# yusong-yan/MultiRaft

Hardware: AMD Instinct MI355X
Metric: quorum commit decisions/sec @64k groups×5 peers; % HBM roofline (higher is better)
Workload: dtype int32

## Files before the change

multiraft_amd/csrc/mraft_abi_msg.hip:

```cpp
#include <vector>

#include "mraft_engine.h"

using namespace mraft::host;

extern "C" {

int mraft_gather_append_args(mraft_engine *h, const int32_t *slots, const int32_t *peers,
                             int64_t n, mraft_ae_args *out_args, int32_t *item_err, int32_t where) {
  TRY(enter(h));
  if (n < 0 || (n > 0 && (!slots || !peers || !out_args || !item_err)))
    return fail(MRAFT_E_INVAL, "null argument");
  if (n == 0) return MRAFT_OK;
  Stage sg(h, where);
  const int32_t *s = sg.in(slots, n), *p = sg.in(peers, n);
  mraft_ae_args *o = sg.out(out_args, n);
  int32_t *e = sg.out(item_err, n);
  TRY(sg.status());
  mraft::launch_gather_args(dev_of(h), s, p, n, o, e, h->stream);
  return sg.finish();
}

int mraft_handle_append_entries(mraft_engine *h, const mraft_ae_args *args, int64_t n,
                                const int32_t *entry_terms, int64_t n_entry_terms,
                                mraft_ae_reply *replies, int32_t *item_err, int32_t where) {
  return mraft_handle_append_entries_ex(h, args, n, entry_terms, n_entry_terms, replies, nullptr, item_err, where);
}

int mraft_handle_append_entries_ex(mraft_engine *h, const mraft_ae_args *args, int64_t n,
                                   const int32_t *entry_terms, int64_t n_entry_terms,
                                   mraft_ae_reply *replies, mraft_ae_result *results, int32_t *item_err,
                                   int32_t where) {
  TRY(enter(h));
  if (n < 0 || (n > 0 && (!args || !replies || !item_err)))
    return fail(MRAFT_E_INVAL, "null argument");
  if (n > INT32_MAX) return fail(MRAFT_E_INVAL, "n = %lld items exceeds 2^31 - 1", (long long)n);
  if (entry_terms && n_entry_terms < 0) return fail(MRAFT_E_INVAL, "n_entry_terms < 0");
  if (n == 0) return MRAFT_OK;
  TRY(ensure_claim(h));
  Stage sg(h, where);
  const mraft_ae_args *a = sg.in(args, n);
  const int32_t *en = sg.in(entry_terms, entry_terms ? n_entry_terms : 0);
  mraft_ae_reply *r = sg.out(replies, n);
  mraft_ae_result *rs = sg.out(results, n);
  int32_t *e = sg.out(item_err, n);
  TRY(sg.status());
  if (en) {
    claim(h, a, n, nullptr, e);
    mraft::launch_handle_ae_host(dev_of(h), a, n, en, n_entry_terms, r, e, rs, h->stream);
    return sg.finish();
  }
  if (!h->ae_total) TRY(alloc_async(h, &h->ae_total, mraft::kAeTotalWords, "AppendEntries counters", true));
  const size_t nn = (size_t)n;
  mraft::HsArgs ka{};
  ka.s = dev_of(h); ka.args = a; ka.n = n; ka.rep = r; ka.err = e; ka.res = rs;
  ka.total = h->ae_total; ka.claim = h->claim; ka.srcmark = h->srcmark; ka.epoch = h->epoch;
  uint8_t *sethd;
  TRY(scratch(h, kScrAeSoff, nn, &ka.soff));
  TRY(scratch(h, kScrAeSetHead, nn, &sethd));
  ka.sethd = sethd;
  TRY(scratch(h, kScrAeDefer, nn * mraft::kAeStripes, &ka.defer));
  const long long last_nd = hint(h, kHintDeferred);
  const long long gmin = h->defer_grid_min;
  const int grid = (int)(last_nd < gmin ? gmin : last_nd > kDeferGridMax ? kDeferGridMax : last_nd);
  ka.nslot = (int)std::min<int64_t>(grid, std::max<int64_t>(1, kCycSlotWords / h->L));
  void *order;
  TRY(scratch_bytes(h, kScrAeOrder, mraft::ae_order_carve(ka, nullptr), &order));
  mraft::ae_order_carve(ka, order);
  TRY(scratch_zeroed(h, kScrAeKin, nn, &ka.kin));
  ka.hint = h->dhint_dev;
  if (h->stage_auto) {
    const long long need = hint(h, kHintStageNeed);
    if (need > h->stage_cap)
      h->stage_cap = std::min<int64_t>((int64_t)INT32_MAX, (need + need / 4 + kStageStep - 1) / kStageStep * kStageStep);
  }
  if (h->stage_cap > 0 && scratch(h, kScrAeStage, (size_t)h->stage_cap, &ka.stage) != MRAFT_OK) {
    ka.stage = nullptr;
    h->stage_auto = false;
  }
  ka.stage_cap = ka.stage ? h->stage_cap : 0;
  const int ni = h->P - 1 < 1 ? 1 : h->P - 1 > 7 ? 7 : h->P - 1;
  const int64_t n_log = gp_of(h) * h->L;
  mraft::launch_claim_ae(a, n, n_log, h->L, gp_of(h), ni, h->claim, h->srcmark, h->epoch, e, sethd, h->ae_total,
                         h->stream);
  mraft::launch_handle_ae_ref(ka, ni, grid, h->stream);
  return sg.finish();
}

int mraft_set_stage_capacity(mraft_engine *h, int64_t words) {
  TRY(enter(h));
  if (words == MRAFT_STAGE_AUTO) {
    h->stage_auto = true;
    return MRAFT_OK;
  }
  if (words < 0 || words > INT32_MAX) return fail(MRAFT_E_INVAL, "stage capacity %lld out of [0, 2^31)", (long long)words);
  h->stage_cap = words;
  h->stage_auto = false;
  return MRAFT_OK;
}

int64_t mraft_get_stage_capacity(const mraft_engine *h) { return h ? h->stage_cap : -1; }

int mraft_process_append_replies(mraft_engine *h, const mraft_ae_result *items, int64_t n,
                                 const int64_t *seg_begin, int64_t n_seg, int32_t *out_flags,
                                 int32_t *item_err, int32_t where) {
  return fold_replies(h, items, n, seg_begin, n_seg, out_flags, item_err, where, [=](const FoldBufs<mraft_ae_result> &b) -> int {
    void *sc;
    TRY(scratch_bytes(h, kScrFoldScan, mraft::fold_scan_bytes(n, b.ns), &sc));
    mraft::launch_fold(dev_of(h), b.it, n, b.sb, b.ns, gp_of(h), h->claim, h->epoch, b.se, b.fl, b.e, sc, h->stream);
    return MRAFT_OK;
  });
}

int mraft_start(mraft_engine *h, const int32_t *slots, const int32_t *counts, int64_t n,
                int32_t *out_index, int32_t *out_term, int32_t *out_is_leader, int32_t *item_err,
                int32_t where) {
  TRY(enter(h));
  if (n < 0 || (n > 0 && (!slots || !out_index || !out_term || !out_is_leader || !item_err)))
    return fail(MRAFT_E_INVAL, "null argument");
  if (n == 0) return MRAFT_OK;
  TRY(ensure_claim(h));
  Stage sg(h, where);
  const int32_t *s = sg.in(slots, n), *c = sg.in(counts, n);
  int32_t *oi = sg.out(out_index, n), *ot = sg.out(out_term, n), *ol = sg.out(out_is_leader, n);
  int32_t *e = sg.out(item_err, n);
  TRY(sg.status());
  mraft::launch_start(dev_of(h), s, c, n, oi, ot, ol, e, h->claim, h->epoch, h->stream);
  return sg.finish();
}

int mraft_collect_apply(mraft_engine *h, int32_t *out_from, int32_t *out_to, int32_t *out_snap_index,
                        int32_t *out_snap_term, int32_t where) {
  TRY(enter(h));
  if (!out_from || !out_to) return fail(MRAFT_E_INVAL, "null argument");
  if (!out_snap_index != !out_snap_term) return fail(MRAFT_E_INVAL, "snapshot outputs: both or neither");
  Stage sg(h, where);
  const size_t gp = (size_t)gp_of(h);
  int32_t *f = sg.out(out_from, gp), *t = sg.out(out_to, gp);
  int32_t *si = sg.out(out_snap_index, gp), *st = sg.out(out_snap_term, gp);
  TRY(sg.status());
  mraft::launch_collect_apply(dev_of(h), f, t, si, st, h->stream);
  return sg.finish();
}

int mraft_collect_apply_compact(mraft_engine *h, int32_t *out_slots, int32_t *out_snap_index,
                                int32_t *out_snap_term, int32_t *out_from, int32_t *out_to, int64_t cap,
                                int64_t *out_n, int32_t where) {
  TRY(enter(h));
  if (cap < 0 || !out_n || (cap > 0 && (!out_slots || !out_from || !out_to)) ||
      (!out_snap_index) != (!out_snap_term))
    return fail(MRAFT_E_INVAL, "null argument");
  Stage sg(h, where);
  int32_t *sl = sg.out(out_slots, cap), *si = sg.out(out_snap_index, cap), *stm = sg.out(out_snap_term, cap);
  int32_t *f = sg.out(out_from, cap), *t = sg.out(out_to, cap), *bc;
  int64_t *total = sg.out(out_n, 1);
  TRY(sg.status());
  TRY(scratch(h, kScrApplyBlocks, (size_t)((gp_of(h) + 255) / 256), &bc));
  mraft::launch_collect_apply_compact(dev_of(h), bc, cap, sl, si, stm, f, t, total, h->stream);
  return sg.finish();
}

int mraft_snapshot(mraft_engine *h, const int32_t *slots, const int32_t *index, int64_t n,
                   int32_t *item_err, int32_t where) {
  TRY(enter(h));
  if (n < 0 || (n > 0 && (!slots || !index || !item_err))) return fail(MRAFT_E_INVAL, "null argument");
  if (n == 0) return MRAFT_OK;
  TRY(ensure_claim(h));
  Stage sg(h, where);
  const int32_t *s = sg.in(slots, n), *x = sg.in(index, n);
  int32_t *e = sg.out(item_err, n);
  TRY(sg.status());
  claim(h, s, n, nullptr, e);
  mraft::launch_snapshot(dev_of(h), s, x, n, e, h->stream);
  return sg.finish();
}

int mraft_gather_install_snapshot_args(mraft_engine *h, const int32_t *slots, const int32_t *peers,
                                       int64_t n, mraft_is_args *out_args, int32_t *item_err,
// ... 184 lines not shown
```

multiraft_amd/csrc/mraft_engine.h:

```cpp
#pragma once
#include <hip/hip_runtime.h>

#include <cstddef>
#include <cstdint>

#include "../../include/mraft.h"
#include "mraft_device.h"
#include "mraft_internal.h"

constexpr int kMaxShards = 8;
constexpr int64_t kDefaultStageWords = (int64_t)1 << 22;
#ifndef MRAFT_DEFER_GRID_MIN
#define MRAFT_DEFER_GRID_MIN 512
#endif
constexpr int kDeferGridMin = MRAFT_DEFER_GRID_MIN;
constexpr int kDeferGridMax = 1 << 16;
constexpr long long kLiteGridMin = 2048;
constexpr long long kLiteGridUnknown = 8192;
constexpr int kAutoProbe = 32;
enum Hint {
  kHintDeferred,
  kHintStageNeed,
  kHintLite,
  kHintWords = kHintLite + kMaxShards
};
constexpr int kStageMax = 7;
enum ScratchSlot {
  kScrTickCount,
  kScrSegErr,
  kScrFoldScan,
  kScrPersistSlots,
  kScrPersistHdr,
  kScrPersistTerms,
  kScrRestoreErr,
  kScrApplyBlocks,
  kScrAeSoff,
  kScrAeSetHead,
  kScrAeStage,
  kScrAeDefer,
  kScrAeOrder,
  kScrAeKin,
  kScrClockLp,
  kScrClockGf,
  kScrClockCommit,
  kScrClockTl,
  kScrClockTg,
  kScrTickerCnt,
  kScrStage0,
  kScrSlots = kScrStage0 + kStageMax
};
constexpr int64_t kStageStep = (int64_t)1 << 20;
#ifndef MRAFT_CYC_SLOT_WORDS
#define MRAFT_CYC_SLOT_WORDS ((int64_t)1 << 25)
#endif
constexpr int64_t kCycSlotWords = MRAFT_CYC_SLOT_WORDS;

struct mraft_engine {
  int32_t G = 0, P = 0, L = 0, device = 0;
  bool owned = false, bound = false;
  mraft_soa dev{};
  hipStream_t own_stream = nullptr, caller_stream = nullptr, stream = nullptr;
  hipStream_t fanin_own = nullptr, fanin_masked = nullptr, tick_masked = nullptr;
  hipEvent_t fanin_ev = nullptr;
  int32_t fan_cus = 0;
  int32_t nshards = 1;
  hipStream_t shard_q[kMaxShards] = {};
  hipEvent_t shard_ev[kMaxShards] = {};
  hipEvent_t fork_ev = nullptr;
  bool shards_pending = false;
  unsigned long long *claim = nullptr;
  uint32_t *srcmark = nullptr;
  uint32_t epoch = 0;
  unsigned long long *ae_total = nullptr;
  int64_t stage_cap = kDefaultStageWords;
  bool stage_auto = true;
  volatile long long *dhint = nullptr;
  long long *dhint_dev = nullptr;
  long long defer_grid_min = kDeferGridMin;
  int32_t tick_mode = MRAFT_TICK_AUTO;
  int32_t *lite_list = nullptr;
  unsigned *lite_cnt = nullptr;
  int lite_par[kMaxShards] = {};
  int auto_since[kMaxShards] = {};
  int32_t *tm_ed = nullptr, *tm_hd = nullptr;
  mraft_timer_config tcfg{};
  uint8_t *reach = nullptr;
  void *scratch_ptr[kScrSlots] = {};
  size_t scratch_cap[kScrSlots] = {};
};

namespace mraft {
namespace host __attribute__((visibility("hidden"))) {

int fail(int code, const char *fmt, ...) __attribute__((format(printf, 2, 3)));

#define HIP_TRY(expr)                                                                   \
  do {                                                                                  \
    hipError_t e_ = (expr);                                                             \
    if (e_ != hipSuccess)                                                               \
      return fail(MRAFT_E_HIP, "%s failed: %s", #expr, hipGetErrorString(e_));          \
  } while (0)

#define TRY(expr)          \
  do {                     \
    int rc_ = (expr);      \
    if (rc_) return rc_;   \
  } while (0)

int join_shards(mraft_engine *h);
int alloc_bytes(mraft_engine *h, void **p, size_t bytes, const char *what);
int scratch_bytes(mraft_engine *h, ScratchSlot slot, size_t bytes, void **out, bool *grew = nullptr);
int ensure_claim(mraft_engine *h);
int copy_array(mraft_engine *h, bool load, int32_t *eng, int32_t *usr, size_t bytes, int32_t where);
int finish_copies(mraft_engine *h, int32_t where);

int launch_tick(mraft_engine *h, const int32_t *lp, int32_t *gf, int32_t *ec, int32_t *et,
                const StartIO *sio = nullptr);

inline int have_handle(const mraft_engine *h) { return h ? MRAFT_OK : fail(MRAFT_E_INVAL, "null engine handle"); }

inline int enter_handle(const mraft_engine *h) {
  TRY(have_handle(h));
  HIP_TRY(hipSetDevice(h->device));
  return MRAFT_OK;
}

inline int enter_tick(mraft_engine *h) {
  TRY(enter_handle(h));
  if (!h->bound) return fail(MRAFT_E_NOSTATE, "engine has no device state bound");
  return MRAFT_OK;
}

inline int enter(mraft_engine *h) {
  TRY(enter_tick(h));
  return join_shards(h);
}

inline long long hint(const mraft_engine *h, int k) { return h->dhint[k]; }

inline int64_t gp_of(const mraft_engine *h) { return (int64_t)h->G * h->P; }

inline Dev dev_of(const mraft_engine *h) {
  Dev d;
  d.term = h->dev.current_term; d.voted = h->dev.voted_for; d.role = h->dev.state;
  d.commit = h->dev.commit_index; d.applied = h->dev.last_applied; d.dummy = h->dev.dummy_index;
  d.last = h->dev.last_index; d.votes = h->dev.granted_votes; d.log = h->dev.log_term;
  d.match = h->dev.match_index; d.next = h->dev.next_index; d.pdirty = h->dev.persist_dirty;
  d.head = h->dev.log_head; d.hsnap = h->dev.has_snapshot; d.srt = h->dev.terms_sorted;
  d.G = h->G; d.P = h->P; d.L = h->L;
  return d;
}

inline Dev dev_slice(const mraft_engine *h, int32_t g0, int32_t g1) {
  Dev d = dev_of(h);
  const int64_t s0 = (int64_t)g0 * h->P;
  for (int32_t **p : {&d.term, &d.voted, &d.role, &d.commit, &d.applied, &d.dummy, &d.last, &d.votes, &d.pdirty,
                      &d.head, &d.hsnap, &d.srt})
    if (*p) *p += s0;
  d.log += s0 * h->L;
  d.match += s0 * h->P;
  d.next += s0 * h->P;
  d.G = g1 - g0;
  return d;
}

template <class T>
int alloc_async(mraft_engine *h, T **p, size_t n, const char *what, bool zero = false) {
  void *v = nullptr;
  const int rc = alloc_bytes(h, &v, sizeof(T) * n, what);
  *p = (T *)v;
  if (rc == MRAFT_OK && zero) HIP_TRY(hipMemsetAsync(v, 0, sizeof(T) * n, h->stream));
  return rc;
}

template <class T>
int scratch(mraft_engine *h, ScratchSlot slot, size_t n, T **out) {
  void *p = nullptr;
  const int rc = scratch_bytes(h, slot, sizeof(T) * n, &p);
  *out = (T *)p;
  return rc;
}

template <class T>
int scratch_zeroed(mraft_engine *h, ScratchSlot slot, size_t n, T **out) {
  void *p = nullptr;
  bool grew = false;
  TRY(scratch_bytes(h, slot, sizeof(T) * n, &p, &grew));
  if (grew) HIP_TRY(hipMemsetAsync(p, 0, h->scratch_cap[slot], h->stream));
  *out = (T *)p;
  return MRAFT_OK;
}

struct Stage {
  mraft_engine *h;
// ... 93 lines not shown
```

multiraft_amd/csrc/mraft_engine.hip:

```cpp
#include <hip/hip_ext.h>

#include <cstdarg>
#include <cstdio>
#include <cstdlib>
#include <string>
#include <vector>

#include "mraft_engine.h"

namespace mraft::host {

namespace {
thread_local std::string g_err;
}

int fail(int code, const char *fmt, ...) {
  char buf[512];
  va_list ap;
  va_start(ap, fmt);
  vsnprintf(buf, sizeof buf, fmt, ap);
  va_end(ap);
  g_err = buf;
  return code;
}

int join_shards(mraft_engine *h) {
  if (!h->shards_pending) return MRAFT_OK;
  for (int s = 0; s < h->nshards; ++s) {
    HIP_TRY(hipEventRecord(h->shard_ev[s], h->shard_q[s]));
    HIP_TRY(hipStreamWaitEvent(h->stream, h->shard_ev[s], 0));
  }
  h->shards_pending = false;
  return MRAFT_OK;
}

int alloc_bytes(mraft_engine *h, void **p, size_t bytes, const char *what) {
  *p = nullptr;
  if (hipMallocAsync(p, bytes, h->stream) != hipSuccess || !*p) {
    (void)hipGetLastError();
    return fail(MRAFT_E_NOMEM, "%s: device allocation of %zu B failed", what, bytes);
  }
  return MRAFT_OK;
}

int scratch_bytes(mraft_engine *h, ScratchSlot slot, size_t bytes, void **out, bool *grew) {
  if (bytes == 0) bytes = 16;
  const bool grows = h->scratch_cap[slot] < bytes;
  if (grows) {
    if (h->scratch_ptr[slot]) HIP_TRY(hipFreeAsync(h->scratch_ptr[slot], h->stream));
    h->scratch_cap[slot] = 0;
    TRY(alloc_bytes(h, &h->scratch_ptr[slot], bytes, "scratch"));
    h->scratch_cap[slot] = bytes;
  }
  if (grew) *grew = grows;
  *out = h->scratch_ptr[slot];
  return MRAFT_OK;
}

int ensure_claim(mraft_engine *h) {
  const size_t gp = (size_t)gp_of(h);
  if (!h->claim) {
    TRY(alloc_async(h, &h->claim, gp, "claim", true));
    TRY(alloc_async(h, &h->srcmark, gp, "srcmark", true));
  }
  if (++h->epoch == 0) {
    HIP_TRY(hipMemsetAsync(h->claim, 0, gp * sizeof *h->claim, h->stream));
    HIP_TRY(hipMemsetAsync(h->srcmark, 0, gp * sizeof *h->srcmark, h->stream));
    if (h->scratch_ptr[kScrAeKin])
      HIP_TRY(hipMemsetAsync(h->scratch_ptr[kScrAeKin], 0, h->scratch_cap[kScrAeKin], h->stream));
    h->epoch = 1;
  }
  return MRAFT_OK;
}

int copy_array(mraft_engine *h, bool load, int32_t *eng, int32_t *usr, size_t bytes, int32_t where) {
  if (!usr) return MRAFT_OK;
  const hipMemcpyKind k = where != MRAFT_HOST ? hipMemcpyDeviceToDevice : load ? hipMemcpyHostToDevice : hipMemcpyDeviceToHost;
  HIP_TRY(hipMemcpyAsync(load ? eng : usr, load ? usr : eng, bytes, k, h->stream));
  return MRAFT_OK;
}

int finish_copies(mraft_engine *h, int32_t where) {
  if (where == MRAFT_HOST) HIP_TRY(hipStreamSynchronize(h->stream));
  return MRAFT_OK;
}

}

using namespace mraft::host;

namespace {

struct ArrDesc { int32_t *mraft_soa::*ptr; int kind; };
const ArrDesc kArrays[] = {
    {&mraft_soa::current_term, 0}, {&mraft_soa::voted_for, 0},   {&mraft_soa::state, 0},
    {&mraft_soa::commit_index, 0}, {&mraft_soa::last_applied, 0}, {&mraft_soa::dummy_index, 0},
    {&mraft_soa::last_index, 0},   {&mraft_soa::granted_votes, 0}, {&mraft_soa::log_term, 1},
    {&mraft_soa::match_index, 2},  {&mraft_soa::next_index, 2},  {&mraft_soa::persist_dirty, 0},
    {&mraft_soa::log_head, 0},     {&mraft_soa::has_snapshot, 0}, {&mraft_soa::terms_sorted, 0}};

size_t arr_bytes(const mraft_engine *h, int kind) {
  int64_t gp = gp_of(h);
  int64_t n = kind == 0 ? gp : kind == 1 ? gp * h->L : gp * h->P;
  return (size_t)n * sizeof(int32_t);
}

void select_stream(mraft_engine *h) {
  h->stream = h->caller_stream ? h->caller_stream : h->tick_masked ? h->tick_masked : h->own_stream;
}

void drain(mraft_engine *h) {
  (void)hipStreamSynchronize(h->stream);
  for (int s = 0; s < h->nshards; ++s)
    if (h->shard_q[s]) (void)hipStreamSynchronize(h->shard_q[s]);
  h->shards_pending = false;
}

int make_queue(mraft_engine *h, bool tick_side, hipStream_t *out) {
  hipDeviceProp_t prop;
  HIP_TRY(hipGetDeviceProperties(&prop, h->device));
  const int ncu = prop.multiProcessorCount, nw = (ncu + 31) / 32;
  std::vector<uint32_t> mask(nw, 0);
  for (int cu = 0; cu < ncu; ++cu)
    if ((cu >= ncu - h->fan_cus) != tick_side) mask[cu / 32] |= 1u << (cu % 32);
  HIP_TRY(hipExtStreamCreateWithCUMask(out, (uint32_t)nw, mask.data()));
  return MRAFT_OK;
}

int destroy_masked(mraft_engine *h, hipStream_t *s) {
  const hipStream_t gone = *s;
  if (!gone) return MRAFT_OK;
  HIP_TRY(hipStreamSynchronize(gone));
  *s = nullptr;
  select_stream(h);
  HIP_TRY(hipStreamDestroy(gone));
  return MRAFT_OK;
}
// ... 27 lines not shown
    if (p) (void)hipFree(p);
    h->dev.*(a.ptr) = nullptr;
  }
  h->owned = false;
  h->bound = false;
}

int create_parts(mraft_engine *h, uint32_t flags) {
  if (flags & MRAFT_CREATE_DEDICATED_QUEUE)
    TRY(make_queue(h, true, &h->own_stream));
  else if (hipStreamCreateWithFlags(&h->own_stream, hipStreamNonBlocking) != hipSuccess)
    return fail(MRAFT_E_HIP, "hipStreamCreate failed");
  h->stream = h->own_stream;
  void *hp = nullptr, *dp = nullptr;
  if (hipHostMalloc(&hp, sizeof(long long) * kHintWords, hipHostMallocMapped) != hipSuccess)
    return fail(MRAFT_E_NOMEM, "pinned host word allocation failed");
  h->dhint = (volatile long long *)hp;
  h->dhint[kHintDeferred] = 0;
  h->dhint[kHintStageNeed] = 0;
  for (int s = 0; s < kMaxShards; ++s) h->dhint[kHintLite + s] = -1;
  if (hipHostGetDevicePointer(&dp, hp, 0) != hipSuccess) return fail(MRAFT_E_HIP, "hipHostGetDevicePointer failed");
  h->dhint_dev = (long long *)dp;
  if (flags & MRAFT_CREATE_NO_ALLOC) return MRAFT_OK;
  h->owned = true;
  for (const auto &a : kArrays)
    if (hipMalloc(&(h->dev.*(a.ptr)), arr_bytes(h, a.kind)) != hipSuccess)
      return fail(MRAFT_E_NOMEM, "device state allocation failed (G=%d P=%d L=%d)", h->G, h->P, h->L);
  h->bound = true;
  (void)hipMemsetAsync(h->dev.log_term, 0, arr_bytes(h, 1), h->stream);
  (void)hipMemsetAsync(h->dev.match_index, 0, arr_bytes(h, 2), h->stream);
  (void)hipMemsetAsync(h->dev.next_index, 0, arr_bytes(h, 2), h->stream);
  mraft::launch_init_state(dev_of(h), h->stream);
  const hipError_t e = hipStreamSynchronize(h->stream);
  if (e != hipSuccess) return fail(MRAFT_E_HIP, "init failed: %s", hipGetErrorString(e));
  return MRAFT_OK;
}

void teardown(mraft_engine *h) {
  (void)hipSetDevice(h->device);
  if (h->stream) drain(h);
  free_owned(h);
  if (h->stream) {
    for (void *p : h->scratch_ptr)
      if (p) (void)hipFreeAsync(p, h->stream);
    for (void *p : {(void *)h->claim, (void *)h->srcmark, (void *)h->ae_total, (void *)h->lite_list,
                    (void *)h->lite_cnt, (void *)h->tm_ed, (void *)h->tm_hd, (void *)h->reach})
      if (p) (void)hipFreeAsync(p, h->stream);
    (void)hipStreamSynchronize(h->stream);
  }
  if (h->fanin_own) (void)hipStreamSynchronize(h->fanin_own);
  if (h->fanin_masked) (void)hipStreamSynchronize(h->fanin_masked);
  destroy_shard_queues(h);
  for (hipStream_t s : {h->own_stream, h->fanin_own, h->fanin_masked, h->tick_masked})
    if (s) (void)hipStreamDestroy(s);
  if (h->fanin_ev) (void)hipEventDestroy(h->fanin_ev);
  if (h->fork_ev) (void)hipEventDestroy(h->fork_ev);
  if (h->dhint) (void)hipHostFree((void *)h->dhint);
  delete h;
}

}

extern "C" {

const char *mraft_last_error_string(void) { return g_err.c_str(); }
int mraft_abi_version(void) { return MRAFT_ABI_VERSION; }

int mraft_create(int32_t groups, int32_t peers, int32_t log_capacity, int32_t device,
                 uint32_t flags, mraft_engine **out) {
  if (!out) return fail(MRAFT_E_INVAL, "out is null");
  *out = nullptr;
  if (groups < 1 || peers < 1 || peers > 8 || log_capacity < 1 || log_capacity > MRAFT_MAX_LOG_CAPACITY)
    return fail(MRAFT_E_INVAL, "bad dims G=%d P=%d L=%d (need G>=1, 1<=P<=8, 1<=L<=%d)", groups, peers,
                log_capacity, MRAFT_MAX_LOG_CAPACITY);
  if ((int64_t)groups * peers > INT32_MAX)
    return fail(MRAFT_E_INVAL, "G*P must fit in int32");
  HIP_TRY(hipSetDevice(device));
  mraft_engine *h = new mraft_engine();
  h->G = groups; h->P = peers; h->L = log_capacity; h->device = device;
  if (const char *e = getenv("MRAFT_DEFER_GRID_MIN")) {
    const long long v = atoll(e);
    if (v >= 1 && v <= kDeferGridMax) h->defer_grid_min = v;
  }
  const int rc = create_parts(h, flags);
  if (rc) {
    teardown(h);
    return rc;
  }
  *out = h;
  return MRAFT_OK;
}

int mraft_destroy(mraft_engine *h) {
  if (h) teardown(h);
  return MRAFT_OK;
}

int mraft_set_stream(mraft_engine *h, void *stream) {
  TRY(enter_handle(h));
  TRY(join_shards(h));
  const hipStream_t old = h->stream, old_caller = h->caller_stream;
  h->caller_stream = (hipStream_t)stream == h->tick_masked ? nullptr : (hipStream_t)stream;
  select_stream(h);
  if (h->stream != old) {
    hipEvent_t ev = nullptr;
    hipError_t e = hipEventCreateWithFlags(&ev, hipEventDisableTiming);
    if (e == hipSuccess) {
      e = hipEventRecord(ev, old);
      if (e == hipSuccess) e = hipStreamWaitEvent(h->stream, ev, 0);
      (void)hipEventDestroy(ev);
    }
    if (e != hipSuccess) {
      h->caller_stream = old_caller;
      select_stream(h);
      return fail(MRAFT_E_HIP, "ordering the new stream: %s", hipGetErrorString(e));
    }
  }
  return MRAFT_OK;
}

void *mraft_get_stream(mraft_engine *h) {
  if (have_handle(h)) return nullptr;
  if (h->shards_pending) {
    if (hipSetDevice(h->device) != hipSuccess) {
      fail(MRAFT_E_HIP, "hipSetDevice failed");
      return nullptr;
    }
    if (join_shards(h) != MRAFT_OK) return nullptr;
  }
  return (void *)h->stream;
}

int mraft_synchronize(mraft_engine *h) {
  TRY(enter_handle(h));
  TRY(join_shards(h));
  HIP_TRY(hipStreamSynchronize(h->stream));
  return MRAFT_OK;
}

int mraft_dims(const mraft_engine *h, int32_t *g, int32_t *p, int32_t *l) {
  TRY(enter_handle(h));
  if (g) *g = h->G;
  if (p) *p = h->P;
  if (l) *l = h->L;
  return MRAFT_OK;
}

int mraft_load_state(mraft_engine *h, const mraft_soa *src, int32_t where) {
  TRY(enter(h));
  if (!src) return fail(MRAFT_E_INVAL, "src is null");
  for (const auto &a : kArrays)
    if (!(src->*(a.ptr))) return fail(MRAFT_E_INVAL, "load_state: every array is required");
  for (const auto &a : kArrays) TRY(copy_array(h, true, h->dev.*(a.ptr), src->*(a.ptr), arr_bytes(h, a.kind), where));
  mraft::launch_terms_sorted(dev_of(h), h->stream);
  HIP_TRY(hipGetLastError());
  return finish_copies(h, where);
}

int mraft_store_state(mraft_engine *h, const mraft_soa *dst, int32_t where) {
  TRY(enter(h));
  if (!dst) return fail(MRAFT_E_INVAL, "dst is null");
  for (const auto &a : kArrays) TRY(copy_array(h, false, h->dev.*(a.ptr), dst->*(a.ptr), arr_bytes(h, a.kind), where));
  return finish_copies(h, where);
}

int mraft_state_view(mraft_engine *h, mraft_soa *out) {
// ... 103 lines not shown
```

multiraft_amd/csrc/mraft_handle_ae.h:

```cpp
#pragma once
#include "mraft_device.h"
#include "mraft_internal.h"
#include "mraft_pass.h"
#include "mraft_rules.h"

namespace mraft {
namespace {

constexpr int kStripes = kAeStripes;
static_assert(16 + 2 * kStripes * 16 == kAeTotalWords, "the counter buffer's layout (mraft_internal.h)");

struct AeKey {
  int64_t row;
  int base;
  int end;
};

__device__ __forceinline__ bool ae_ref_ok(const mraft_ae_args &a, int64_t n_log, int L) {
  return !(a.n_entries < 0 || a.entries_offset < 0 || a.entries_offset + a.n_entries > n_log ||
           a.entries_offset % L + a.n_entries > L);
}

__device__ __forceinline__ bool ae_index_ok(const mraft_ae_args &a) {
  return index_in_domain((int64_t)a.prev_log_index + a.n_entries);
}

__device__ __forceinline__ AeKey ae_key(const mraft_ae_args &a, int64_t gp, int64_t n_log, int L) {
  if (a.slot < 0 || a.slot >= gp || !ae_ref_ok(a, n_log, L) || !ae_index_ok(a)) return AeKey{-1, 0, 0};
  return AeKey{a.entries_offset / L, (int)(a.entries_offset % L) - (a.prev_log_index + 1),
               a.prev_log_index + a.n_entries};
}

__device__ __forceinline__ bool same_key(const AeKey &x, const AeKey &y) {
  return x.row >= 0 && x.row == y.row && x.base == y.base && x.end == y.end;
}

enum : int { AE_DEFER = -1, AE_NONE = 0, AE_DONE, AE_BAD, AE_STALE, AE_BELOW, AE_MISS, AE_MERGE };
enum : int {
  HM_MAIN = 0,
  HM_DEFER = 1,
  HM_HOST = 2,
  HM_ORDER = 3
};

#ifndef MRAFT_AE_MINW
#define MRAFT_AE_MINW 8
#endif
#ifndef MRAFT_AE_DMINW
#define MRAFT_AE_DMINW 7
#endif

__device__ __forceinline__ void mark_persist_ae(const Dev &s, int64_t slot, int bits) {
  if (s.pdirty && bits) (void)__hip_atomic_fetch_or(&s.pdirty[slot], bits, __ATOMIC_RELAXED, __HIP_MEMORY_SCOPE_AGENT);
}

__device__ __forceinline__ HsArgs reload_hs() {
  const __attribute__((address_space(4))) HsArgs *kp =
      (const __attribute__((address_space(4))) HsArgs *)__builtin_amdgcn_kernarg_segment_ptr();
  asm volatile("" : "+s"(kp));
  HsArgs k;
  k.s.term = kp->s.term; k.s.voted = kp->s.voted; k.s.role = kp->s.role; k.s.commit = kp->s.commit;
  k.s.applied = kp->s.applied; k.s.dummy = kp->s.dummy; k.s.last = kp->s.last; k.s.votes = kp->s.votes;
  k.s.log = kp->s.log; k.s.match = kp->s.match; k.s.next = kp->s.next; k.s.pdirty = kp->s.pdirty;
  k.s.head = kp->s.head; k.s.hsnap = kp->s.hsnap; k.s.srt = kp->s.srt; k.s.G = kp->s.G; k.s.P = kp->s.P; k.s.L = kp->s.L;
  k.args = kp->args; k.n = kp->n; k.ent0 = kp->ent0; k.n_ent0 = kp->n_ent0; k.stage = kp->stage;
  k.stage_cap = kp->stage_cap; k.soff = kp->soff; k.sethd = kp->sethd; k.defer = kp->defer; k.total = kp->total;
  k.claim = kp->claim; k.srcmark = kp->srcmark; k.epoch = kp->epoch; k.fb = kp->fb; k.kin = kp->kin;
  k.cslot = kp->cslot; k.nslot = kp->nslot; k.cyc = kp->cyc; k.hint = kp->hint;
  k.rep = kp->rep; k.err = kp->err; k.res = kp->res;
  return k;
}

__device__ __forceinline__ int4 no_record() {
  int m = -1, z = 0;
  asm volatile("" : "+v"(m), "+v"(z));
  return make_int4(m, m, z, z);
}

__device__ __forceinline__ int lanes_below(unsigned long long m) {
  return (int)__builtin_amdgcn_mbcnt_hi((uint32_t)(m >> 32), __builtin_amdgcn_mbcnt_lo((uint32_t)m, 0u));
}

__device__ __forceinline__ int at_load(int32_t *p) {
  return __hip_atomic_load(p, __ATOMIC_RELAXED, __HIP_MEMORY_SCOPE_AGENT);
}
__device__ __forceinline__ void at_store(int32_t *p, int v) {
  __hip_atomic_store(p, v, __ATOMIC_RELAXED, __HIP_MEMORY_SCOPE_AGENT);
}
__device__ __forceinline__ void wave_fence() {
  __builtin_amdgcn_fence(__ATOMIC_SEQ_CST, "workgroup");
  __builtin_amdgcn_s_waitcnt(0);
}

__device__ __forceinline__ void tag_inc(unsigned long long *p, uint32_t epoch) {
  unsigned long long old = __hip_atomic_load(p, __ATOMIC_RELAXED, __HIP_MEMORY_SCOPE_AGENT);
  for (;;) {
    const unsigned long long nv =
        (uint32_t)(old >> 32) == epoch ? old + 1 : (((unsigned long long)epoch << 32) | 1ull);
    if (__hip_atomic_compare_exchange_strong(p, &old, nv, __ATOMIC_RELAXED, __ATOMIC_RELAXED,
                                             __HIP_MEMORY_SCOPE_AGENT))
      return;
  }
}
__device__ __forceinline__ int tag_count(const unsigned long long *p, uint32_t epoch) {
  const unsigned long long v = __hip_atomic_load(p, __ATOMIC_RELAXED, __HIP_MEMORY_SCOPE_AGENT);
  return (uint32_t)(v >> 32) == epoch ? (int)(uint32_t)v : 0;
}

__device__ __forceinline__ void defer_lanes(const HsArgs &k0, bool dfr, bool stg, int64_t i, int n, const int32_t *row,
                                            int head, int from, int L, int wraw) {
  const unsigned long long m = __ballot(dfr);
  const int lane = lane_id(), q0 = first_lane(m);
  const int x = (int)(blockIdx.x & (kStripes - 1));
  unsigned long long b = 0;
  if (lane == q0) b = atomicAdd(&k0.total[kAeCntDeferred + kAeCntStripe * x], (unsigned long long)__popcll(m));
  b = ((unsigned long long)(uint32_t)__builtin_amdgcn_readlane((int)(b >> 32), q0) << 32) |
      (uint32_t)__builtin_amdgcn_readlane((int)(uint32_t)b, q0);
  if (dfr) {
    k0.defer[x * k0.n + (int64_t)b + lanes_below(m)] = i;
    int64_t in_place = -2;
    asm volatile("" : "+v"(in_place));
    if (!stg) k0.soff[i] = in_place;
    k0.fb[i] = make_int4(wraw, 0, 0, 0);
    if (wraw >= 0) tag_inc(&k0.kin[wraw], k0.epoch);
  }
  const unsigned long long smask = __ballot(stg);
  if (!smask) return;
  const int64_t cap8 = k0.stage_cap / kStripes;
  int64_t pre = stg ? (int64_t)n : 0;
#pragma unroll
  for (int o = 1; o < 64; o <<= 1) {
    const int64_t v = __shfl_up(pre, o, 64);
    if (lane >= o) pre += v;
  }
  const int64_t tot = __shfl(pre, 63, 64);
  unsigned long long sb = 0;
  if (lane == first_lane(smask)) sb = atomicAdd(&k0.total[kAeCntStaged + kAeCntStripe * x], (unsigned long long)tot);
  sb = ((unsigned long long)(uint32_t)__builtin_amdgcn_readlane((int)(sb >> 32), first_lane(smask)) << 32) |
       (uint32_t)__builtin_amdgcn_readlane((int)(uint32_t)sb, first_lane(smask));
  const int64_t my = (int64_t)sb + pre - (stg ? (int64_t)n : 0);
  if (stg) k0.soff[i] = x * cap8 + my;
  for (unsigned long long sm = smask; sm; sm &= sm - 1) {
    const int q = first_lane(sm);
    const int nq = __builtin_amdgcn_readlane(n, q);
    const int64_t oq = ((int64_t)__builtin_amdgcn_readlane((int)((uint64_t)my >> 32), q) << 32) |
                       (uint32_t)__builtin_amdgcn_readlane((int)(uint32_t)my, q);
    const long long o = x * cap8 + oq;
    if (oq + nq <= cap8) {
      const uint64_t ra = (uint64_t)(uintptr_t)row;
      const int32_t *rq = (const int32_t *)(uintptr_t)(((uint64_t)(uint32_t)__builtin_amdgcn_readlane((int)(ra >> 32), q) << 32) |
                                                      (uint32_t)__builtin_amdgcn_readlane((int)(uint32_t)ra, q));
      wave_copy_from_ring(rq, 0, __builtin_amdgcn_readlane(head, q), L, __builtin_amdgcn_readlane(from, q),
                          k0.stage + o, nq);
    }
  }
}

template <int NI, int MODE>
__device__ __forceinline__ void handle_one(const HsArgs &k0, int64_t first, int size, int64_t so_force = -2) {
  const Dev &s = k0.s;
  const mraft_ae_args *__restrict__ args = k0.args;
  const int lane = lane_id();
  const bool mine = lane < size;
  int64_t i = first + (mine ? lane : 0);
  const int e = mine ? k0.err[i] : 1;
  mraft_ae_args a = args[i];
  const int64_t so0 = MODE == HM_DEFER ? k0.soff[i] : so_force;
  asm volatile("" ::"v"(a.slot), "v"(a.term), "v"(a.prev_log_index), "v"(a.prev_log_term),
               "v"(a.n_entries), "v"(a.leader_commit), "v"(a.entries_offset), "v"(so0));
  int L = s.L;
  asm volatile("" : "+s"(L));
  const int64_t gp = (int64_t)s.G * s.P;
  int f = a.slot;
  const int prev = a.prev_log_index, nn = a.n_entries;
  int fterm = 0, fdummy = 0, flast = 0, fc = 0, fhead = 0;
  if (!e) { fterm = s.term[f]; fdummy = s.dummy[f]; flast = s.last[f]; fc = s.commit[f]; fhead = s.head[f]; }
  RingRow src = flat_src(k0.ent0, 0, prev);
  int64_t n_ent = k0.n_ent0;
  bool ok = true, dup = false, dfr = false, stg = false;
  int64_t srow = 0;
  int rhead = 0;
  unsigned long long cr = 0;
  if (MODE == HM_HOST) {
    if (!e) src = flat_src(k0.ent0, a.entries_offset, prev);
  } else if (!e) {
    ok = ae_ref_ok(a, gp * L, L);
    srow = ok ? a.entries_offset / L : 0;
    unsigned long long cs = 0;
    uint32_t sm = 0;
    if (MODE == HM_MAIN) {
      cs = k0.claim[f];
      sm = k0.srcmark[f];
      if (ok && nn > 0) cr = k0.claim[srow];
    }
    if (ok && srow < gp) rhead = s.head[srow];
    if (MODE == HM_MAIN) {
      dup = !claim_won(cs, k0.epoch, i);
      dfr = !dup && ok && sm == k0.epoch;
      stg = dfr && nn > 0 && (uint32_t)(cr >> 32) == k0.epoch;
    }
    const int64_t so = MODE == HM_MAIN ? -2 : so0;
    if (so >= 0) {
      src = flat_src(k0.stage, so, prev);
      n_ent = k0.stage_cap;
      a.entries_offset = so;
    } else {
      src.p = s.log;
      src.row = srow * L;
      src.L = L;
      src.base = rhead + (int)(a.entries_offset % L) - (prev + 1);
      n_ent = INT64_MAX;
    }
  }
  int cls = e ? AE_NONE : AE_DONE;
  if (dup) cls = AE_NONE;
  else if (dfr) cls = AE_DEFER;
  else if (!e && (!ok || nn < 0 || a.entries_offset < 0 || !ae_index_ok(a) ||
                  (nn > 0 && src.L == INT32_MAX && a.entries_offset + nn > n_ent)))
    cls = AE_BAD;
  const bool live = cls == AE_DONE;
  if (dup && mine) k0.err[i] = MRAFT_ITEM_DUP_SLOT;
  if (MODE == HM_MAIN && __ballot(dfr)) {
    const int wraw = (nn > 0 && ae_index_ok(a) && (uint32_t)(cr >> 32) == k0.epoch) ? claim_index(cr) : -1;
    defer_lanes(k0, dfr, stg, i, nn, s.log + srow * L, rhead, (int)(a.entries_offset % L), L, wraw);
  }
  if (k0.res && mine && cls != AE_DEFER) {
    int PP = s.P;
    asm volatile("" : "+s"(PP));
    int4 *rr = reinterpret_cast<int4 *>(k0.res + i);
    rr[0] = live ? make_int4((f / PP) * PP + a.leader_id, f % PP, a.term, prev) : no_record();
  }
  const bool claim = live && nn > 0 && (a.flags & MRAFT_AE_ENTRIES_SORTED) != 0;
  const bool claim0 = claim && a.prev_log_term <= *src.at(prev + 1);
  mraft_ae_reply r = {0, 0, 0, 0};
  int ftp = 0;
  if (live) {
    if (a.term < fterm) {
      cls = AE_STALE;
      r.term = fterm;
    } else if (prev < fdummy) {
      cls = AE_BELOW;
      r.conflict_index = fdummy + 1;
    } else {
      ftp = prev > flast ? 0 : s.log[(int64_t)f * L + ring(prev - fdummy + fhead, L)];
      if (prev > flast || ftp != a.prev_log_term) {
        cls = AE_MISS;
        r.term = a.term;
        if (prev > flast) r.conflict_index = flast + 1;
        else r.conflict_index = prev;
      } else {
        cls = AE_MERGE;
      }
    }
  }
  for (unsigned long long m = __ballot(cls == AE_MISS && prev <= flast && prev > fdummy + 1); m; m &= m - 1) {
    const int q = first_lane(m);
    const int qf = __shfl(f, q, 64), qd = __shfl(fdummy, q, 64), qh = __shfl(fhead, q, 64),
              qp = __shfl(prev, q, 64), qa = __shfl(ftp, q, 64);
    const int ci = wave_conflict_scan(s.log + (int64_t)uni(qf) * L, uni(qd), uni(qh), L, uni(qp), uni(qa));
    if (lane == q) r.conflict_index = ci;
  }
  int newlast = -1, fcommit_new = -1, srt_new = -1;
  const int merge_m = (int)(__ballot(cls == AE_MERGE) & ((1ull << NI) - 1));
  int shint = claim0 ? (prev == fdummy ? 1 : 0) : -1;
  if (merge_m) {
    Fol<NI, true> fo;
    fo.log = s.log;
    fo.slot0 = 0;
    fo.skip = NI;
    fo.L = L;
    fo.cmp = merge_m;
    fo.copy = 0;
    fo.capok = (int)(__ballot(cls == AE_MERGE && (int64_t)prev + nn - fdummy <= (int64_t)L - 1) & ((1ull << NI) - 1));
    fo.full = 0;
    const int phi = uni(__shfl(prev + nn, first_lane((unsigned long long)merge_m), 64));
    int plo = phi + 1;
#pragma unroll
    for (int q = 0; q < NI; ++q)
      if ((merge_m >> q) & 1) plo = min(plo, uni(__shfl(prev, q, 64)) + 1);
    const int B = pass_bias(plo);
    const int pl = plo - B, ph = phi - B, nend = ph + 1;
    const int q0 = first_lane((unsigned long long)merge_m);
    RingRow ss;
    {
      const uint64_t pa = (uint64_t)(uintptr_t)src.p;
      const uint32_t lo = (uint32_t)__shfl((int)(uint32_t)pa, q0, 64), hi = (uint32_t)__shfl((int)(pa >> 32), q0, 64);
      ss.p = (const int32_t *)(uintptr_t)(((uint64_t)uni((int)hi) << 32) | (uint32_t)uni((int)lo));
      const uint64_t ra = (uint64_t)src.row;
      const uint32_t rlo = (uint32_t)__shfl((int)(uint32_t)ra, q0, 64), rhi = (uint32_t)__shfl((int)(ra >> 32), q0, 64);
      ss.row = (long long)(((uint64_t)uni((int)rhi) << 32) | (uint32_t)uni((int)rlo));
      ss.base = uni(__shfl(src.base, q0, 64)) + B;
      ss.L = uni(__shfl(src.L, q0, 64));
    }
    bool vec = (L & 3) == 0 && ((uintptr_t)s.log & 15) == 0;
#pragma unroll
    for (int q = 0; q < NI; ++q) {
      fo.slot[q] = uni(__shfl(f, q, 64));
      const int sp = uni(__shfl(prev, q, 64)), sl = uni(__shfl(flast, q, 64));
      fo.base[q] = 0; fo.start[q] = 0; fo.cend[q] = 0;
      fo.cfrom[q] = 0;
      if ((merge_m >> q) & 1) {
        fo.base[q] = uni(__shfl(fhead - fdummy, q, 64)) + B;
        fo.start[q] = sp + 1 - B;
        fo.cend[q] = min(phi, sl) + 1 - B;
        vec = vec && ((((uintptr_t)ss.at(fo.start[q]) ^ (uintptr_t)fo.at(q, fo.start[q])) & 15) == 0);
      }
    }
    if (ss.L == INT32_MAX) {
      const uint64_t nb = (uint64_t)n_ent;
      const uint32_t nlo = (uint32_t)__shfl((int)(uint32_t)nb, q0, 64), nhi = (uint32_t)__shfl((int)(nb >> 32), q0, 64);
      const int64_t sn = (int64_t)(((uint64_t)uni((int)nhi) << 32) | (uint32_t)uni((int)nlo));
      vec = vec && (((uintptr_t)ss.at(pl)) & ~(uintptr_t)15) >= (uintptr_t)ss.p &&
            (((uintptr_t)ss.at(ph)) | 15) < (uintptr_t)(ss.p + sn);
    }
    vec = __ballot(!vec) == 0;
    int found = -1;
    DescTrack dt{__ballot(cls == AE_MERGE && claim0) != 0, 0, INT32_MIN};
    __shared__ int stash[12][64];
    stash[0][lane] = cls; stash[1][lane] = f; stash[2][lane] = fterm; stash[3][lane] = flast;
    stash[4][lane] = fc; stash[5][lane] = a.term; stash[6][lane] = a.leader_commit;
    stash[7][lane] = r.conflict_index; stash[8][lane] = r.term;
    stash[9][lane] = (int)(uint32_t)(uint64_t)i; stash[10][lane] = (int)((uint64_t)i >> 32);
    stash[11][lane] = shint;
    asm volatile("" ::: "memory");
    if (vec) {
      int c = pl - (int)(((uintptr_t)ss.at(pl) >> 2) & 31);
      if (c <= ph && fo.cmp) c = pass_pipe<false>(ss, fo, nend, 1, 0, 0, found, c, pl, ph, dt);
      copy_loop<true, false>(ss, fo, c, nend, pl, ph, 1, 0, 0, found, dt);
    } else {
      int c = pl;
      for (; c <= ph && fo.cmp; c += 256) pass_chunk<1, false, false>(ss, fo, nend, 1, 0, 0, found, c, pl, ph, dt);
      copy_loop<false, false>(ss, fo, c, nend, pl, ph, 1, 0, 0, found, dt);
    }
    asm volatile("" ::: "memory");
    cls = stash[0][lane]; f = stash[1][lane]; fterm = stash[2][lane]; flast = stash[3][lane];
    fc = stash[4][lane]; a.term = stash[5][lane]; a.leader_commit = stash[6][lane];
    r.conflict_index = stash[7][lane]; r.term = stash[8][lane];
    i = (int64_t)(((uint64_t)(uint32_t)stash[10][lane] << 32) | (uint32_t)stash[9][lane]);
    shint = stash[11][lane];
    const HsArgs kr = reload_hs();
    int32_t *__restrict__ err = kr.err;
    mraft_ae_reply *__restrict__ rep = kr.rep;
#pragma unroll
    for (int q = 0; q < NI; ++q) {
      if (lane != q || cls != AE_MERGE) continue;
      if ((fo.full >> q) & 1) {
        cls = AE_DONE;
        err[i] = MRAFT_ITEM_LOG_FULL;
        rep[i] = r;
      } else {
        int last_after = flast;
        if (fo.cfrom[q] > 0) {
          newlast = last_after = phi;
          if (dt.last > fo.start[q]) shint = -1;
          srt_new = shint < 0 ? 0 : (shint == 1 && fo.cfrom[q] == fo.start[q] ? 1 : -1);
        }
        if (a.leader_commit > fc) fcommit_new = min(a.leader_commit, last_after);
        r.term = a.term; r.success = 1;
      }
    }
  }
  const HsArgs kt = reload_hs();
  const Dev &s2 = kt.s;
  int32_t *__restrict__ err2 = kt.err;
  mraft_ae_reply *__restrict__ rep2 = kt.rep;
  if (cls == AE_NONE) {
    if (mine) rep2[i] = r;
  } else if (cls == AE_BAD) {
    rep2[i] = r;
    err2[i] = MRAFT_ITEM_BAD_SLOT;
  } else if (cls == AE_STALE) {
    rep2[i] = r;
    mark_persist_ae(s2, f, MRAFT_PERSIST_STATE);
  } else if (cls >= AE_BELOW) {
    if (a.term > fterm) { s2.term[f] = a.term; s2.voted[f] = -1; }
    s2.role[f] = kFollower;
    if (newlast >= 0) s2.last[f] = newlast;
    if (srt_new >= 0) s2.srt[f] = srt_new;
    if (fcommit_new >= 0) s2.commit[f] = fcommit_new;
    mark_persist_ae(s2, f, MRAFT_PERSIST_STATE);
    rep2[i] = r;
  }
  mraft_ae_result *__restrict__ res = kt.res;
  if (res && mine && cls != AE_DEFER) {
    int4 *rr = reinterpret_cast<int4 *>(res + i);
    if (cls == AE_DONE) rr[0] = no_record();
    rr[1] = cls >= AE_STALE ? make_int4(nn, r.term, r.success, r.conflict_index) : make_int4(0, 0, 0, 0);
  }
}

}
}
```

Before: 24.80 million.

## Fuse deferred entry staging into merge pass and bound stage growth by free memory

Staging copies of deferred append-entries, which used to be done per lane inside defer_lanes with a serial loop over staged lanes, now go into the main merge pass. Staged lanes are handled as extra copy targets through a FolStage wrapper and a new stage_copy_loop that streams the source once and writes to both log rows and stage slots. Separately, auto-growth of the stage buffer is now capped by a ceiling derived from free device memory. A new scratch_keep allocator keeps the old buffer when an allocation fails. This adds a larger shared stash and more complex copy logic in the hot kernel.

Result: no change. 24.73 million (-0.3%).

```diff
diff --git a/multiraft_amd/csrc/mraft_abi_msg.hip b/multiraft_amd/csrc/mraft_abi_msg.hip
--- a/multiraft_amd/csrc/mraft_abi_msg.hip
+++ b/multiraft_amd/csrc/mraft_abi_msg.hip
@@ -3,6 +3,16 @@
 #include "mraft_engine.h"
 
 using namespace mraft::host;
+
+static int64_t stage_ceiling(const mraft_engine *h) {
+  if (h->stage_ceiling >= 0) return h->stage_ceiling;
+  size_t free_bytes = 0, total_bytes = 0;
+  if (hipMemGetInfo(&free_bytes, &total_bytes) != hipSuccess) {
+    (void)hipGetLastError();
+    return 0;
+  }
+  return stage_ceiling_words(free_bytes);
+}
 
 extern "C" {
 
@@ -69,15 +79,20 @@
   mraft::ae_order_carve(ka, order);
   TRY(scratch_zeroed(h, kScrAeKin, nn, &ka.kin));
   ka.hint = h->dhint_dev;
-  if (h->stage_auto) {
-    const long long need = hint(h, kHintStageNeed);
-    if (need > h->stage_cap)
-      h->stage_cap = std::min<int64_t>((int64_t)INT32_MAX, (need + need / 4 + kStageStep - 1) / kStageStep * kStageStep);
-  }
-  if (h->stage_cap > 0 && scratch(h, kScrAeStage, (size_t)h->stage_cap, &ka.stage) != MRAFT_OK) {
-    ka.stage = nullptr;
+  void *stage = nullptr;
+  if (h->stage_auto && hint(h, kHintStageNeed) > h->stage_cap) {
+    const StageAuto sa = stage_auto_step(h->stage_cap, hint(h, kHintStageNeed), stage_ceiling(h), [&](int64_t words) {
+      return scratch_keep(h, kScrAeStage, sizeof(int32_t) * (size_t)words, &stage) == MRAFT_OK;
+    });
+    h->stage_cap = sa.cap;
+    h->stage_auto = sa.on;
+  }
+  if (h->stage_cap > 0 && scratch_keep(h, kScrAeStage, sizeof(int32_t) * (size_t)h->stage_cap, &stage) != MRAFT_OK) {
+    stage = h->scratch_ptr[kScrAeStage];
+    h->stage_cap = std::min<int64_t>(h->stage_cap, (int64_t)(h->scratch_cap[kScrAeStage] / sizeof(int32_t)));
     h->stage_auto = false;
   }
+  ka.stage = (int32_t *)stage;
   ka.stage_cap = ka.stage ? h->stage_cap : 0;
   const int ni = h->P - 1 < 1 ? 1 : h->P - 1 > 7 ? 7 : h->P - 1;
   const int64_t n_log = gp_of(h) * h->L;
@@ -93,7 +108,7 @@
     h->stage_auto = true;
     return MRAFT_OK;
   }
-  if (words < 0 || words > INT32_MAX) return fail(MRAFT_E_INVAL, "stage capacity %lld out of [0, 2^31)", (long long)words);
+  if (words < 0 || words > kStageMaxWords) return fail(MRAFT_E_INVAL, "stage capacity %lld out of [0, 2^31)", (long long)words);
   h->stage_cap = words;
   h->stage_auto = false;
   return MRAFT_OK;
diff --git a/multiraft_amd/csrc/mraft_engine.h b/multiraft_amd/csrc/mraft_engine.h
--- a/multiraft_amd/csrc/mraft_engine.h
+++ b/multiraft_amd/csrc/mraft_engine.h
@@ -7,6 +7,7 @@
 #include "../../include/mraft.h"
 #include "mraft_device.h"
 #include "mraft_internal.h"
+#include "mraft_stage_policy.h"
 
 constexpr int kMaxShards = 8;
 constexpr int64_t kDefaultStageWords = (int64_t)1 << 22;
@@ -49,7 +50,6 @@
   kScrStage0,
   kScrSlots = kScrStage0 + kStageMax
 };
-constexpr int64_t kStageStep = (int64_t)1 << 20;
 #ifndef MRAFT_CYC_SLOT_WORDS
 #define MRAFT_CYC_SLOT_WORDS ((int64_t)1 << 25)
 #endif
@@ -74,6 +74,7 @@
   unsigned long long *ae_total = nullptr;
   int64_t stage_cap = kDefaultStageWords;
   bool stage_auto = true;
+  int64_t stage_ceiling = -1;
   volatile long long *dhint = nullptr;
   long long *dhint_dev = nullptr;
   long long defer_grid_min = kDeferGridMin;
@@ -110,6 +111,7 @@
 int join_shards(mraft_engine *h);
 int alloc_bytes(mraft_engine *h, void **p, size_t bytes, const char *what);
 int scratch_bytes(mraft_engine *h, ScratchSlot slot, size_t bytes, void **out, bool *grew = nullptr);
+int scratch_keep(mraft_engine *h, ScratchSlot slot, size_t bytes, void **out);
 int ensure_claim(mraft_engine *h);
 int copy_array(mraft_engine *h, bool load, int32_t *eng, int32_t *usr, size_t bytes, int32_t where);
 int finish_copies(mraft_engine *h, int32_t where);
diff --git a/multiraft_amd/csrc/mraft_engine.hip b/multiraft_amd/csrc/mraft_engine.hip
--- a/multiraft_amd/csrc/mraft_engine.hip
+++ b/multiraft_amd/csrc/mraft_engine.hip
@@ -53,6 +53,19 @@
     h->scratch_cap[slot] = bytes;
   }
   if (grew) *grew = grows;
+  *out = h->scratch_ptr[slot];
+  return MRAFT_OK;
+}
+
+int scratch_keep(mraft_engine *h, ScratchSlot slot, size_t bytes, void **out) {
+  if (bytes == 0) bytes = 16;
+  if (h->scratch_cap[slot] < bytes) {
+    void *p = nullptr;
+    TRY(alloc_bytes(h, &p, bytes, "scratch"));
+    if (h->scratch_ptr[slot]) (void)hipFreeAsync(h->scratch_ptr[slot], h->stream);
+    h->scratch_ptr[slot] = p;
+    h->scratch_cap[slot] = bytes;
+  }
   *out = h->scratch_ptr[slot];
   return MRAFT_OK;
 }
@@ -246,6 +259,10 @@
     const long long v = atoll(e);
     if (v >= 1 && v <= kDeferGridMax) h->defer_grid_min = v;
   }
+  if (const char *e = getenv("MRAFT_STAGE_CEILING_WORDS")) {
+    const long long v = atoll(e);
+    if (v >= 0 && v <= kStageMaxWords) h->stage_ceiling = v;
+  }
   const int rc = create_parts(h, flags);
   if (rc) {
     teardown(h);
diff --git a/multiraft_amd/csrc/mraft_handle_ae.h b/multiraft_amd/csrc/mraft_handle_ae.h
--- a/multiraft_amd/csrc/mraft_handle_ae.h
+++ b/multiraft_amd/csrc/mraft_handle_ae.h
@@ -1,4 +1,6 @@
 #pragma once
+#include <type_traits>
+
 #include "mraft_device.h"
 #include "mraft_internal.h"
 #include "mraft_pass.h"
@@ -107,8 +109,7 @@
   return (uint32_t)(v >> 32) == epoch ? (int)(uint32_t)v : 0;
 }
 
-__device__ __forceinline__ void defer_lanes(const HsArgs &k0, bool dfr, bool stg, int64_t i, int n, const int32_t *row,
-                                            int head, int from, int L, int wraw) {
+__device__ __forceinline__ int defer_lanes(const HsArgs &k0, bool dfr, bool stg, int64_t i, int n, int wraw) {
   const unsigned long long m = __ballot(dfr);
   const int lane = lane_id(), q0 = first_lane(m);
   const int x = (int)(blockIdx.x & (kStripes - 1));
@@ -125,7 +126,7 @@
     if (wraw >= 0) tag_inc(&k0.kin[wraw], k0.epoch);
   }
   const unsigned long long smask = __ballot(stg);
-  if (!smask) return;
+  if (!smask) return -1;
   const int64_t cap8 = k0.stage_cap / kStripes;
   int64_t pre = stg ? (int64_t)n : 0;
 #pragma unroll
@@ -140,18 +141,71 @@
        (uint32_t)__builtin_amdgcn_readlane((int)(uint32_t)sb, first_lane(smask));
   const int64_t my = (int64_t)sb + pre - (stg ? (int64_t)n : 0);
   if (stg) k0.soff[i] = x * cap8 + my;
-  for (unsigned long long sm = smask; sm; sm &= sm - 1) {
-    const int q = first_lane(sm);
-    const int nq = __builtin_amdgcn_readlane(n, q);
-    const int64_t oq = ((int64_t)__builtin_amdgcn_readlane((int)((uint64_t)my >> 32), q) << 32) |
-                       (uint32_t)__builtin_amdgcn_readlane((int)(uint32_t)my, q);
-    const long long o = x * cap8 + oq;
-    if (oq + nq <= cap8) {
-      const uint64_t ra = (uint64_t)(uintptr_t)row;
-      const int32_t *rq = (const int32_t *)(uintptr_t)(((uint64_t)(uint32_t)__builtin_amdgcn_readlane((int)(ra >> 32), q) << 32) |
-                                                      (uint32_t)__builtin_amdgcn_readlane((int)(uint32_t)ra, q));
-      wave_copy_from_ring(rq, 0, __builtin_amdgcn_readlane(head, q), L, __builtin_amdgcn_readlane(from, q),
-                          k0.stage + o, nq);
+  return stg && my + n <= cap8 ? (int)(x * cap8 + my) : -1;
+}
+
+template <int NI>
+struct FolStage : Fol<NI, true> {
+  static constexpr int kStaged = INT32_MIN;
+  int32_t *stage;
+  __device__ __forceinline__ int32_t *at(int q, int idx) const {
+    if (this->base[q] == kStaged) {
+      bounds_note(idx);
+      return at_u(stage + ((long long)this->slot[q] - this->start[q]), idx);
+    }
+    return Fol<NI, true>::at(q, idx);
+  }
+};
+
+template <bool VEC, class Src, class F>
+__device__ __forceinline__ void stage_copy_loop(const Src &src, const F &fo, int c, int nend, int plo, int phi,
+                                                DescTrack &dt) {
+  constexpr int NI = F::kNI;
+  constexpr int CW = 256;
+  const int lane = lane_id();
+  int cmask = fo.copy;
+  if (c > phi || !cmask) return;
+  if constexpr (VEC) {
+    int4 cur = make_int4(0, 0, 0, 0);
+    if (c + 4 * lane + 3 >= plo && c + 4 * lane <= phi) cur = ld4(src.at(c + 4 * lane));
+    for (;;) {
+      const int i0 = c + 4 * lane, cn = c + CW;
+      const bool more = cn < nend;
+      int4 nxt = make_int4(0, 0, 0, 0);
+      if (more && cn + 4 * lane <= phi) nxt = ld4(src.at(cn + 4 * lane));
+      const int e[4] = {cur.x, cur.y, cur.z, cur.w};
+      dt.template see<4>(e, c, plo, phi);
+#pragma unroll
+      for (int q = 0; q < NI; ++q) {
+        if (!((cmask >> q) & 1)) continue;
+        if (i0 >= fo.cfrom[q] && i0 + 3 < nend) {
+          st4(fo.at(q, i0), cur.x, cur.y, cur.z, cur.w);
+        } else {
+#pragma unroll
+          for (int u = 0; u < 4; ++u)
+            if (i0 + u >= fo.cfrom[q] && i0 + u < nend) st1(fo.at(q, i0 + u), e[u]);
+        }
+      }
+      if (!more) return;
+      c = cn;
+      cur = nxt;
+    }
+  } else {
+    for (; c <= phi; c += CW) {
+      int idx[4], e[4];
+#pragma unroll
+      for (int u = 0; u < 4; ++u) {
+        idx[u] = c + 64 * u + lane;
+        e[u] = (idx[u] >= plo && idx[u] <= phi) ? ld1(src.at(idx[u])) : 0;
+      }
+      dt.see_strided(e, c, plo, phi);
+#pragma unroll
+      for (int q = 0; q < NI; ++q) {
+        if (!((cmask >> q) & 1)) continue;
+#pragma unroll
+        for (int u = 0; u < 4; ++u)
+          if (idx[u] >= fo.cfrom[q] && idx[u] < nend) st1(fo.at(q, idx[u]), e[u]);
+      }
     }
   }
 }
@@ -172,7 +226,8 @@
   asm volatile("" : "+s"(L));
   const int64_t gp = (int64_t)s.G * s.P;
   int f = a.slot;
-  const int prev = a.prev_log_index, nn = a.n_entries;
+  const int prev = a.prev_log_index;
+  int nn = a.n_entries;
   int fterm = 0, fdummy = 0, flast = 0, fc = 0, fhead = 0;
   if (!e) { fterm = s.term[f]; fdummy = s.dummy[f]; flast = s.last[f]; fc = s.commit[f]; fhead = s.head[f]; }
   RingRow src = flat_src(k0.ent0, 0, prev);
@@ -220,9 +275,12 @@
     cls = AE_BAD;
   const bool live = cls == AE_DONE;
   if (dup && mine) k0.err[i] = MRAFT_ITEM_DUP_SLOT;
+  int stage_m = 0;
+  int sdst = -1;
   if (MODE == HM_MAIN && __ballot(dfr)) {
     const int wraw = (nn > 0 && ae_index_ok(a) && (uint32_t)(cr >> 32) == k0.epoch) ? claim_index(cr) : -1;
-    defer_lanes(k0, dfr, stg, i, nn, s.log + srow * L, rhead, (int)(a.entries_offset % L), L, wraw);
+    sdst = defer_lanes(k0, dfr, stg, i, nn, wraw);
+    stage_m = (int)(__ballot(sdst >= 0 && ae_index_ok(a) && prev >= 0) & ((1ull << NI) - 1));
   }
   if (k0.res && mine && cls != AE_DEFER) {
     int PP = s.P;
@@ -263,24 +321,28 @@
   int newlast = -1, fcommit_new = -1, srt_new = -1;
   const int merge_m = (int)(__ballot(cls == AE_MERGE) & ((1ull << NI) - 1));
   int shint = claim0 ? (prev == fdummy ? 1 : 0) : -1;
-  if (merge_m) {
-    Fol<NI, true> fo;
+  __shared__ int stash[MODE == HM_MAIN ? 13 : 12][64];
+  constexpr bool STAGES = MODE == HM_MAIN;
+  const int pass_m = STAGES ? merge_m | stage_m : merge_m;
+  if (pass_m) {
+    std::conditional_t<STAGES, FolStage<NI>, Fol<NI, true>> fo;
     fo.log = s.log;
+    if constexpr (STAGES) fo.stage = k0.stage;
     fo.slot0 = 0;
     fo.skip = NI;
     fo.L = L;
     fo.cmp = merge_m;
-    fo.copy = 0;
+    fo.copy = STAGES ? stage_m : 0;
     fo.capok = (int)(__ballot(cls == AE_MERGE && (int64_t)prev + nn - fdummy <= (int64_t)L - 1) & ((1ull << NI) - 1));
     fo.full = 0;
-    const int phi = uni(__shfl(prev + nn, first_lane((unsigned long long)merge_m), 64));
+    const int phi = uni(__shfl(prev + nn, first_lane((unsigned long long)pass_m), 64));
     int plo = phi + 1;
 #pragma unroll
     for (int q = 0; q < NI; ++q)
-      if ((merge_m >> q) & 1) plo = min(plo, uni(__shfl(prev, q, 64)) + 1);
+      if ((pass_m >> q) & 1) plo = min(plo, uni(__shfl(prev, q, 64)) + 1);
     const int B = pass_bias(plo);
     const int pl = plo - B, ph = phi - B, nend = ph + 1;
-    const int q0 = first_lane((unsigned long long)merge_m);
+    const int q0 = first_lane((unsigned long long)pass_m);
     RingRow ss;
     {
       const uint64_t pa = (uint64_t)(uintptr_t)src.p;
@@ -305,6 +367,13 @@
         fo.cend[q] = min(phi, sl) + 1 - B;
         vec = vec && ((((uintptr_t)ss.at(fo.start[q]) ^ (uintptr_t)fo.at(q, fo.start[q])) & 15) == 0);
       }
+      if constexpr (STAGES) {
+        if ((stage_m >> q) & 1) {
+          fo.slot[q] = uni(__shfl(sdst, q, 64));
+          fo.base[q] = fo.kStaged;
+          fo.start[q] = fo.cfrom[q] = sp + 1 - B;
+        }
+      }
     }
     if (ss.L == INT32_MAX) {
       const uint64_t nb = (uint64_t)n_ent;
@@ -316,21 +385,23 @@
     vec = __ballot(!vec) == 0;
     int found = -1;
     DescTrack dt{__ballot(cls == AE_MERGE && claim0) != 0, 0, INT32_MIN};
-    __shared__ int stash[12][64];
     stash[0][lane] = cls; stash[1][lane] = f; stash[2][lane] = fterm; stash[3][lane] = flast;
     stash[4][lane] = fc; stash[5][lane] = a.term; stash[6][lane] = a.leader_commit;
     stash[7][lane] = r.conflict_index; stash[8][lane] = r.term;
     stash[9][lane] = (int)(uint32_t)(uint64_t)i; stash[10][lane] = (int)((uint64_t)i >> 32);
     stash[11][lane] = shint;
+    if constexpr (STAGES) stash[12][lane] = nn;
     asm volatile("" ::: "memory");
     if (vec) {
       int c = pl - (int)(((uintptr_t)ss.at(pl) >> 2) & 31);
       if (c <= ph && fo.cmp) c = pass_pipe<false>(ss, fo, nend, 1, 0, 0, found, c, pl, ph, dt);
-      copy_loop<true, false>(ss, fo, c, nend, pl, ph, 1, 0, 0, found, dt);
+      if constexpr (STAGES) stage_copy_loop<true>(ss, fo, c, nend, pl, ph, dt);
+      else copy_loop<true, false>(ss, fo, c, nend, pl, ph, 1, 0, 0, found, dt);
     } else {
       int c = pl;
       for (; c <= ph && fo.cmp; c += 256) pass_chunk<1, false, false>(ss, fo, nend, 1, 0, 0, found, c, pl, ph, dt);
-      copy_loop<false, false>(ss, fo, c, nend, pl, ph, 1, 0, 0, found, dt);
+      if constexpr (STAGES) stage_copy_loop<false>(ss, fo, c, nend, pl, ph, dt);
+      else copy_loop<false, false>(ss, fo, c, nend, pl, ph, 1, 0, 0, found, dt);
     }
     asm volatile("" ::: "memory");
     cls = stash[0][lane]; f = stash[1][lane]; fterm = stash[2][lane]; flast = stash[3][lane];
@@ -338,6 +409,7 @@
     r.conflict_index = stash[7][lane]; r.term = stash[8][lane];
     i = (int64_t)(((uint64_t)(uint32_t)stash[10][lane] << 32) | (uint32_t)stash[9][lane]);
     shint = stash[11][lane];
+    if constexpr (STAGES) nn = stash[12][lane];
     const HsArgs kr = reload_hs();
     int32_t *__restrict__ err = kr.err;
     mraft_ae_reply *__restrict__ rep = kr.rep;
diff --git a/multiraft_amd/csrc/mraft_stage_policy.h b/multiraft_amd/csrc/mraft_stage_policy.h
--- /dev/null
+++ b/multiraft_amd/csrc/mraft_stage_policy.h
@@ -0,0 +1,34 @@
+#pragma once
+#include <algorithm>
+#include <cstddef>
+#include <cstdint>
+
+namespace mraft {
+namespace host {
+
+constexpr int64_t kStageStep = (int64_t)1 << 20;
+constexpr int64_t kStageMaxWords = INT32_MAX;
+constexpr int kStageFreeShare = 2;
+
+inline int64_t stage_ceiling_words(size_t free_bytes) {
+  return std::min<int64_t>(kStageMaxWords, (int64_t)(free_bytes / kStageFreeShare / sizeof(int32_t)));
+}
+
+inline int64_t stage_want(int64_t need) {
+  return std::min<int64_t>(kStageMaxWords, (need + need / 4 + kStageStep - 1) / kStageStep * kStageStep);
+}
+
+struct StageAuto {
+  int64_t cap;
+  bool on;
+};
+template <class TryAlloc>
+StageAuto stage_auto_step(int64_t cap, int64_t need, int64_t ceiling, TryAlloc &&try_alloc) {
+  if (need <= cap) return {cap, true};
+  const int64_t want = stage_want(need);
+  if (want > ceiling || !try_alloc(want)) return {cap, false};
+  return {want, true};
+}
+
+}
+}
```
